# UVA-Computer-Vision-Lab/midvision-probe

Measured on AMD Instinct MI355X. Metric: images/sec feature-extract+probe-step, ViT-B/16 224^2, higher is better.
Workload: dtype f16x2 (compensated fp16 pairs of activations and frozen weights, two f16 MFMA products per contraction, fp32 accumulate, feature error as bf16x3; attention: Q.K^T the same two products over compensated pairs, P.V fp16 probabilities x (fp16 + bf16) V; probe, fp32 residual/LN/softmax/loss as in bf16x3

## Files before the change

midvision-probe_amd/csrc/attention.hip:

```cpp
#include "mvp_common.h"

#ifndef MVP_ATT_NT
#define MVP_ATT_NT 0
#endif
#ifndef MVP_ATT_LD_AUX
#define MVP_ATT_LD_AUX 0
#endif
namespace {

#ifndef MVP_ATT_PRIO
#define MVP_ATT_PRIO 0
#endif
#ifndef MVP_ATT_STAGGER
#define MVP_ATT_STAGGER 0
#endif
#if MVP_ATT_PRIO
#define ATT_PRIO(v) __builtin_amdgcn_s_setprio(v)
#else
#define ATT_PRIO(v)
#endif
#ifndef MVP_ATT_ABLATE
#define MVP_ATT_ABLATE 0
#endif
constexpr int TILE = 64 * 128;
constexpr float ATT_DEFER = 6.0f;

template <int SPLIT>
struct AttnState {
  bf16x8_t q_hi[2][2], q_lo[2][2];
  f32x4_t o_acc[4][2];
  float m_run[2], l_run[2];
};

struct AttnBias {
  const float* row[2];
  float scale;
  const float* rel;
  unsigned qoff[2];
  int Kh, Kw, q16, r16;
};

template <int SPLIT, bool LAST, int VF16 = 0, int BIAS = 0>
__device__ __forceinline__ void attn_tile(AttnState<SPLIT>& st, const char* kb, const char* vb, int key0, int N, float cs, int lane,
                                          const AttnBias& ab = AttnBias{}) {
  static_assert(!VF16 || SPLIT == 3, "the fp16-probability form belongs to the bf16x3 mode");
  const int g = lane >> 4, c16 = lane & 15;
  const int nsub = LAST ? min(4, (N - key0 + 15) >> 4) : 4;
  f32x4_t s[4][2];
#pragma unroll
  for (int t = 0; t < 4; ++t)
#pragma unroll
    for (int qt = 0; qt < 2; ++qt) s[t][qt] = f32x4_t{0.f, 0.f, 0.f, 0.f};
  f32x4_t bv[4][2];
  if constexpr (BIAS == 1) {
#pragma unroll
    for (int t = 0; t < 4; ++t)
#pragma unroll
      for (int qt = 0; qt < 2; ++qt)
        bv[t][qt] = (LAST && t >= nsub) ? f32x4_t{0.f, 0.f, 0.f, 0.f} : *(const f32x4_t*)(ab.row[qt] + key0 + t * 16);
  }
  ATT_PRIO(1);
#pragma unroll
  for (int ks = 0; ks < (MVP_ATT_ABLATE == 3 ? 0 : 2); ++ks) {
    const int coff = (((ks << 2) + g) ^ (lane & 7)) << 4;
#pragma unroll
    for (int t = 0; t < 4; ++t) {
      if (LAST && t >= nsub) continue;
      const char* ka = kb + (t * 16 + c16) * 128 + coff;
      const bf16x8_t k_hi = *(const bf16x8_t*)ka;
      if (VF16 == 2) {
        const f16x8_t k_lo = *(const f16x8_t*)(ka + TILE);
        const f16x8_t k_h = __builtin_bit_cast(f16x8_t, k_hi);
#pragma unroll
        for (int qt = 0; qt < 2; ++qt) {
          s[t][qt] = __builtin_amdgcn_mfma_f32_16x16x32_f16(k_lo, __builtin_bit_cast(f16x8_t, st.q_lo[qt][ks]), s[t][qt], 0, 0, 0);
          s[t][qt] = __builtin_amdgcn_mfma_f32_16x16x32_f16(k_h, __builtin_bit_cast(f16x8_t, st.q_hi[qt][ks]), s[t][qt], 0, 0, 0);
        }
        continue;
      }
      if (SPLIT == 3) {
        const bf16x8_t k_lo = *(const bf16x8_t*)(ka + TILE);
#pragma unroll
        for (int qt = 0; qt < 2; ++qt) {
          s[t][qt] = __builtin_amdgcn_mfma_f32_16x16x32_bf16(k_lo, st.q_hi[qt][ks], s[t][qt], 0, 0, 0);
          s[t][qt] = __builtin_amdgcn_mfma_f32_16x16x32_bf16(k_hi, st.q_lo[qt][ks], s[t][qt], 0, 0, 0);
        }
      }
#pragma unroll
      for (int qt = 0; qt < 2; ++qt)
        s[t][qt] = __builtin_amdgcn_mfma_f32_16x16x32_bf16(k_hi, st.q_hi[qt][ks], s[t][qt], 0, 0, 0);
    }
  }
  ATT_PRIO(0);
  if constexpr (BIAS == 1) {
#pragma unroll
    for (int t = 0; t < 4; ++t)
#pragma unroll
      for (int qt = 0; qt < 2; ++qt)
#pragma unroll
        for (int j = 0; j < 4; ++j) s[t][qt][j] = __builtin_fmaf(s[t][qt][j], ab.scale, bv[t][qt][j]);
  }
  if constexpr (BIAS == 2) {
    unsigned k0 = (unsigned)(key0 + g * 4);
    asm volatile("" : "+v"(k0));
    const unsigned Kw4 = (unsigned)ab.Kw << 2, Kh4 = (unsigned)ab.Kh << 2;
    const unsigned q0y = k0 / (unsigned)ab.Kw;
    unsigned ty = q0y << 2, tx = (k0 - q0y * (unsigned)ab.Kw) << 2;
    const char* base = (const char*)ab.rel;
#pragma unroll
    for (int t = 0; t < 4; ++t) {
      if (!(LAST && t >= nsub)) {
        unsigned ky = ty, kx = tx;
#pragma unroll
        for (int j = 0; j < 4; ++j) {
          const bool dead = LAST && (int)k0 + t * 16 + j >= N;
          const unsigned yy = dead ? 0u : ky, xx = (dead ? 0u : kx) + Kh4;
#pragma unroll
          for (int qt = 0; qt < 2; ++qt)
            s[t][qt][j] = __builtin_fmaf(s[t][qt][j], ab.scale, *(const float*)(base + (ab.qoff[qt] + yy)) + *(const float*)(base + (ab.qoff[qt] + xx)));
          kx += 4;
          if (kx == Kw4) {
            kx = 0;
            ky += 4;
          }
        }
      }
      ty += ab.q16;
      tx += ab.r16;
      if (tx >= Kw4) {
        tx -= Kw4;
        ty += 4;
      }
      __builtin_amdgcn_sched_barrier(0);
    }
  }
  const int kbase = key0 + g * 4;
  bf16x8_t p_hi[2][2], p_lo[2][2];
  f16x8_t p_h[2][2];
#pragma unroll
  for (int qt = 0; qt < 2; ++qt) {
    if (VF16 && MVP_ATT_ABLATE != 1) {
      float tmax = -1e30f;
#pragma unroll
      for (int t = 0; t < 4; ++t)
#pragma unroll
        for (int j = 0; j < 4; ++j) {
          if (LAST) s[t][qt][j] = ((kbase + t * 16 + j) < N) ? s[t][qt][j] : -1e30f;
          tmax = fmaxf(tmax, s[t][qt][j]);
        }
      tmax = fmaxf(tmax, __shfl_xor(tmax, 16, 64));
      tmax = fmaxf(tmax, __shfl_xor(tmax, 32, 64));
      if (__builtin_amdgcn_ballot_w64((tmax - st.m_run[qt]) * cs > ATT_DEFER) != 0) {
        const float m_new = fmaxf(st.m_run[qt], tmax);
        const float alpha = __builtin_amdgcn_exp2f((st.m_run[qt] - m_new) * cs);
        st.m_run[qt] = m_new;
        st.l_run[qt] *= alpha;
#pragma unroll
        for (int dt = 0; dt < 4; ++dt) st.o_acc[dt][qt] *= alpha;
      }
      const float mc = st.m_run[qt] * cs;
      float psum = 0.f;
#pragma unroll
      for (int t = 0; t < 4; ++t)
#pragma unroll
        for (int j = 0; j < 4; ++j) {
          const float pv = (LAST && t >= nsub) ? 0.f : __builtin_amdgcn_exp2f(s[t][qt][j] * cs - mc);
          psum += pv;
          p_h[qt][t >> 1][(t & 1) * 4 + j] = (_Float16)pv;
          p_lo[qt][t >> 1][(t & 1) * 4 + j] = (__bf16)pv;
        }
      st.l_run[qt] += psum;
      continue;
    }
    if (MVP_ATT_ABLATE == 1) {
#pragma unroll
      for (int t = 0; t < 4; ++t)
#pragma unroll
        for (int j = 0; j < 4; ++j) {
          p_hi[qt][t >> 1][(t & 1) * 4 + j] = (__bf16)s[t][qt][j];
          if (SPLIT == 3) p_lo[qt][t >> 1][(t & 1) * 4 + j] = (__bf16)(s[t][qt][j] * cs);
        }
      st.l_run[qt] = 1.f;
      continue;
    }
    float tmax = -1e30f;
#pragma unroll
    for (int t = 0; t < 4; ++t)
#pragma unroll
      for (int j = 0; j < 4; ++j) {
        if (LAST) s[t][qt][j] = ((kbase + t * 16 + j) < N) ? s[t][qt][j] : -1e30f;
        tmax = fmaxf(tmax, s[t][qt][j]);
      }
    tmax = fmaxf(tmax, __shfl_xor(tmax, 16, 64));
    tmax = fmaxf(tmax, __shfl_xor(tmax, 32, 64));
    const float m_new = fmaxf(st.m_run[qt], tmax);
    const float alpha = __builtin_amdgcn_exp2f((st.m_run[qt] - m_new) * cs);
    const float mc = m_new * cs;
    st.m_run[qt] = m_new;
    float psum = 0.f;
#pragma unroll
    for (int t = 0; t < 4; ++t)
#pragma unroll
      for (int j = 0; j < 4; ++j) {
        const float pv = (LAST && t >= nsub) ? 0.f : __builtin_amdgcn_exp2f(s[t][qt][j] * cs - mc);
        psum += pv;
        const __bf16 ph = (__bf16)pv;
        p_hi[qt][t >> 1][(t & 1) * 4 + j] = ph;
        if (SPLIT == 3) p_lo[qt][t >> 1][(t & 1) * 4 + j] = (__bf16)(pv - (float)ph);
      }
    st.l_run[qt] = st.l_run[qt] * alpha + psum;
#pragma unroll
    for (int dt = 0; dt < 4; ++dt) st.o_acc[dt][qt] *= alpha;
  }
  const int tr_q = c16 >> 2, tr_p = lane & 3;
  ATT_PRIO(1);
#pragma unroll
  for (int ks = 0; ks < (MVP_ATT_ABLATE == 2 ? 0 : 2); ++ks) {
    if (LAST && 2 * ks >= nsub) continue;
    const int row = ks * 32 + g * 4 + tr_q;
    const int fsw = ((row >> 1) & 3) << 1;
#pragma unroll
    for (int dt = 0; dt < 4; ++dt) {
      const int off = row * 128 + ((((dt << 1) + (tr_p >> 1)) ^ fsw) << 4) + ((tr_p & 1) << 3);
      const bf16x4_t a0 = __builtin_amdgcn_ds_read_tr16_b64_v4bf16((__attribute__((address_space(3))) bf16x4_t*)(vb + off));
      const bf16x4_t a1 = __builtin_amdgcn_ds_read_tr16_b64_v4bf16((__attribute__((address_space(3))) bf16x4_t*)(vb + off + 16 * 128));
      const bf16x8_t v_hi = __builtin_shufflevector(a0, a1, 0, 1, 2, 3, 4, 5, 6, 7);
      if (VF16) {
        const bf16x4_t b0 = __builtin_amdgcn_ds_read_tr16_b64_v4bf16((__attribute__((address_space(3))) bf16x4_t*)(vb + TILE + off));
        const bf16x4_t b1 = __builtin_amdgcn_ds_read_tr16_b64_v4bf16((__attribute__((address_space(3))) bf16x4_t*)(vb + TILE + off + 16 * 128));
        const bf16x8_t v_lo = __builtin_shufflevector(b0, b1, 0, 1, 2, 3, 4, 5, 6, 7);
        const f16x8_t v_h = __builtin_bit_cast(f16x8_t, v_hi);
#pragma unroll
        for (int qt = 0; qt < 2; ++qt) {
          st.o_acc[dt][qt] = __builtin_amdgcn_mfma_f32_16x16x32_bf16(v_lo, p_lo[qt][ks], st.o_acc[dt][qt], 0, 0, 0);
          st.o_acc[dt][qt] = __builtin_amdgcn_mfma_f32_16x16x32_f16(v_h, p_h[qt][ks], st.o_acc[dt][qt], 0, 0, 0);
        }
        continue;
      }
      if (SPLIT == 3) {
        const bf16x4_t b0 = __builtin_amdgcn_ds_read_tr16_b64_v4bf16((__attribute__((address_space(3))) bf16x4_t*)(vb + TILE + off));
        const bf16x4_t b1 = __builtin_amdgcn_ds_read_tr16_b64_v4bf16((__attribute__((address_space(3))) bf16x4_t*)(vb + TILE + off + 16 * 128));
        const bf16x8_t v_lo = __builtin_shufflevector(b0, b1, 0, 1, 2, 3, 4, 5, 6, 7);
#pragma unroll
        for (int qt = 0; qt < 2; ++qt) {
          st.o_acc[dt][qt] = __builtin_amdgcn_mfma_f32_16x16x32_bf16(v_lo, p_hi[qt][ks], st.o_acc[dt][qt], 0, 0, 0);
          st.o_acc[dt][qt] = __builtin_amdgcn_mfma_f32_16x16x32_bf16(v_hi, p_lo[qt][ks], st.o_acc[dt][qt], 0, 0, 0);
        }
      }
#pragma unroll
      for (int qt = 0; qt < 2; ++qt)
        st.o_acc[dt][qt] = __builtin_amdgcn_mfma_f32_16x16x32_bf16(v_hi, p_hi[qt][ks], st.o_acc[dt][qt], 0, 0, 0);
    }
  }
  ATT_PRIO(0);
}

template <int SPLIT>
__device__ __forceinline__ void attn_load_q(AttnState<SPLIT>& st, const mvp_attention_args& p, size_t rowbase, int q0, int h, int lane) {
  const int g = lane >> 4, c16 = lane & 15;
#pragma unroll
  for (int qt = 0; qt < 2; ++qt) {
    const int qrow = min(q0 + qt * 16 + c16, p.N - 1);
    const size_t off = (rowbase + qrow) * p.ld_qkv + h * 64 + g * 8;
#pragma unroll
    for (int ks = 0; ks < 2; ++ks) {
      st.q_hi[qt][ks] = *(const bf16x8_t*)(p.qkv_hi + off + ks * 32);
      if (SPLIT == 3) st.q_lo[qt][ks] = *(const bf16x8_t*)(p.qkv_lo + off + ks * 32);
    }
  }
#pragma unroll
  for (int i = 0; i < 4; ++i)
#pragma unroll
    for (int j = 0; j < 2; ++j) st.o_acc[i][j] = f32x4_t{0.f, 0.f, 0.f, 0.f};
  st.m_run[0] = st.m_run[1] = -1e30f;
  st.l_run[0] = st.l_run[1] = 0.f;
}

template <int SPLIT>
__device__ __forceinline__ void attn_store(AttnState<SPLIT>& st, const mvp_attention_args& p, size_t rowbase, int q0, int h, int lane) {
  const int g = lane >> 4, c16 = lane & 15;
#pragma unroll
  for (int qt = 0; qt < 2; ++qt) {
    float l = st.l_run[qt];
    l += __shfl_xor(l, 16, 64);
    l += __shfl_xor(l, 32, 64);
    const float inv = 1.0f / l;
    const int qrow = q0 + qt * 16 + c16;
    if (qrow >= p.N) continue;
    const bool ilv = p.out_layout == MVP_PAIR_A_ILV32;
    const size_t ob = (rowbase + qrow) * p.ld_out + (ilv ? h * 128 : h * 64) + g * 4;
#pragma unroll
    for (int dt = 0; dt < 4; ++dt) {
      uint32_t h01, l01, h23, l23;
      if (p.out_f16) {
        split2_f16_comp(st.o_acc[dt][qt][0] * inv, st.o_acc[dt][qt][1] * inv, h01, l01);
        split2_f16_comp(st.o_acc[dt][qt][2] * inv, st.o_acc[dt][qt][3] * inv, h23, l23);
      } else {
        split2_bf16(st.o_acc[dt][qt][0] * inv, st.o_acc[dt][qt][1] * inv, h01, l01);
        split2_bf16(st.o_acc[dt][qt][2] * inv, st.o_acc[dt][qt][3] * inv, h23, l23);
      }
      if (ilv) {
        const size_t o = ob + (dt >> 1) * 64 + (dt & 1) * 16;
        store_out((u32x2_t*)(p.out_hi + o), u32x2_t{h01, h23}, MVP_ATT_NT);
        store_out((u32x2_t*)(p.out_hi + o + 32), u32x2_t{l01, l23}, MVP_ATT_NT);
      } else {
        store_out((u32x2_t*)(p.out_hi + ob + dt * 16), u32x2_t{h01, h23}, MVP_ATT_NT);
        if (p.out_lo) store_out((u32x2_t*)(p.out_lo + ob + dt * 16), u32x2_t{l01, l23}, MVP_ATT_NT);
      }
    }
  }
}

template <int SPLIT>
__device__ __forceinline__ void attn_stage_piece(const mvp_attention_args& p, size_t rowbase, int h, int key0, int r, char* kdst, char* vdst, int lane) {
  const int rsub = lane >> 3;
  const int kc = ((lane & 7) ^ rsub) << 3;
  const int vc = ((lane & 7) ^ (((lane >> 4) & 3) << 1)) << 3;
  const int HD = p.H * 64;
  if (MVP_ATT_ABLATE == 4) return;
  const int krow = min(key0 + r + rsub, p.N - 1);
  const size_t ro = (rowbase + krow) * p.ld_qkv + h * 64;
  __builtin_amdgcn_global_load_lds(GLB_PTR(p.qkv_hi + ro + HD + kc), LDS_PTR(kdst + r * 128), 16, 0, MVP_ATT_LD_AUX);
  __builtin_amdgcn_global_load_lds(GLB_PTR(p.qkv_hi + ro + 2 * HD + vc), LDS_PTR(vdst + r * 128), 16, 0, MVP_ATT_LD_AUX);
  if (SPLIT == 3) {
    __builtin_amdgcn_global_load_lds(GLB_PTR(p.qkv_lo + ro + HD + kc), LDS_PTR(kdst + TILE + r * 128), 16, 0, MVP_ATT_LD_AUX);
    __builtin_amdgcn_global_load_lds(GLB_PTR(p.qkv_lo + ro + 2 * HD + vc), LDS_PTR(vdst + TILE + r * 128), 16, 0, MVP_ATT_LD_AUX);
  }
}

template <int BIAS> struct AttnKArgs { typedef mvp_attention_args type; };
template <> struct AttnKArgs<1> { typedef mvp_attention_bias_args type; };
template <> struct AttnKArgs<2> { typedef mvp_attention_relpos_args type; };
__host__ __device__ __forceinline__ const mvp_attention_args& att_of(const mvp_attention_args& a) { return a; }
__host__ __device__ __forceinline__ const mvp_attention_args& att_of(const mvp_attention_bias_args& a) { return a.att; }
__host__ __device__ __forceinline__ const mvp_attention_args& att_of(const mvp_attention_relpos_args& a) { return a.att; }
__device__ __forceinline__ void attn_bias_rows(AttnBias& ab, const mvp_attention_bias_args& a, int bh, int h, int q0, int lane) {
  const int g = lane >> 4, c16 = lane & 15;
#pragma unroll
  for (int qt = 0; qt < 2; ++qt)
    ab.row[qt] = a.bias + (size_t)h * (size_t)a.bias_head_stride + (size_t)min(q0 + qt * 16 + c16, a.att.N - 1) * (size_t)a.ld_bias + g * 4;
}
__device__ __forceinline__ void attn_bias_rows(AttnBias& ab, const mvp_attention_relpos_args& a, int bh, int h, int q0, int lane) {
  const int c16 = lane & 15;
#pragma unroll
  for (int qt = 0; qt < 2; ++qt) ab.qoff[qt] = ((unsigned)min(q0 + qt * 16 + c16, a.att.N - 1) * (unsigned)a.ld_rel) << 2;
}
__device__ __forceinline__ void attn_bias_rows(AttnBias&, const mvp_attention_args&, int, int, int, int) {}
__device__ __forceinline__ void attn_bias_pair(AttnBias& ab, const mvp_attention_relpos_args& a, int bh) { ab.rel = a.rel + (size_t)bh * (size_t)a.rel_bh_stride; }
__device__ __forceinline__ void attn_bias_pair(AttnBias&, const mvp_attention_bias_args&, int) {}
__device__ __forceinline__ void attn_bias_pair(AttnBias&, const mvp_attention_args&, int) {}
__device__ __forceinline__ void attn_bias_init(AttnBias& ab, const mvp_attention_relpos_args& a) {
  ab.Kh = a.Kh;
  ab.Kw = a.Kw;
  ab.q16 = (16 / a.Kw) << 2;
  ab.r16 = (16 % a.Kw) << 2;
}
__device__ __forceinline__ void attn_bias_init(AttnBias&, const mvp_attention_bias_args&) {}
__device__ __forceinline__ void attn_bias_init(AttnBias&, const mvp_attention_args&) {}

template <int SPLIT, int VF16 = 0, int BIAS = 0>
__global__ __launch_bounds__(256) void attention_stream_kernel(const typename AttnKArgs<BIAS>::type pa) {
  const mvp_attention_args& p = att_of(pa);
  f16_saturate_mode();
  extern __shared__ __attribute__((aligned(16))) char smem[];
  constexpr int NARR = (SPLIT == 3) ? 2 : 1;
  constexpr int STAGE = 2 * NARR * TILE;
  const int lane = threadIdx.x & 63, wave = threadIdx.x >> 6;
  const int bh = blockIdx.y, b = bh / p.H, h = bh - b * p.H;
  const int q0 = blockIdx.x * 128 + wave * 32;
  const int nkt = (p.N + 63) >> 6;
  const size_t rowbase = (size_t)b * p.N;
  AttnState<SPLIT> st;
  attn_load_q<SPLIT>(st, p, rowbase, q0, h, lane);
  const float cs = BIAS ? 1.44269504088896340736f : p.scale * 1.44269504088896340736f;
  const bool active = q0 < p.N;
  AttnBias ab{};
  if constexpr (BIAS != 0) {
    ab.scale = p.scale;
    attn_bias_init(ab, pa);
    attn_bias_pair(ab, pa, bh);
    if (active) attn_bias_rows(ab, pa, bh, h, q0, lane);
  }

  auto stage = [&](int buf, int kt) {
    char* base = smem + buf * STAGE;
#pragma unroll
    for (int ps = 0; ps < 2; ++ps) attn_stage_piece<SPLIT>(p, rowbase, h, kt * 64, ps * 32 + wave * 8, base, base + NARR * TILE, lane);
  };
  stage(0, 0);
  asm volatile("s_waitcnt vmcnt(0)" ::: "memory");
  __syncthreads();
  for (int kt = 0; kt < nkt; ++kt) {
    if (kt + 1 < nkt) stage((kt + 1) & 1, kt + 1);
    if (active) {
      const char* kb = smem + (kt & 1) * STAGE;
      if (kt == nkt - 1) attn_tile<SPLIT, true, VF16, BIAS>(st, kb, kb + NARR * TILE, kt * 64, p.N, cs, lane, ab);
      else attn_tile<SPLIT, false, VF16, BIAS>(st, kb, kb + NARR * TILE, kt * 64, p.N, cs, lane, ab);
    }
    asm volatile("s_waitcnt vmcnt(0)" ::: "memory");
    __syncthreads();
  }
  if (active) attn_store<SPLIT>(st, p, rowbase, q0, h, lane);
}

template <int SPLIT, int VF16 = 0, int BIAS = 0>
__global__ __launch_bounds__(512) void attention_resident_kernel(const typename AttnKArgs<BIAS>::type pa) {
  const mvp_attention_args& p = att_of(pa);
  f16_saturate_mode();
  extern __shared__ __attribute__((aligned(16))) char smem[];
  constexpr int NARR = (SPLIT == 3) ? 2 : 1;
  constexpr int STAGE = 2 * NARR * TILE;
  const int lane = threadIdx.x & 63, wave = threadIdx.x >> 6;
  const int q0 = wave * 32;
  const int nkt = (p.N + 63) >> 6, nslot = nkt + 1;
  const int npair = p.B * p.H;
  const float cs = BIAS ? 1.44269504088896340736f : p.scale * 1.44269504088896340736f;
  const bool active = q0 < p.N;
  const int g = lane >> 4, c16 = lane & 15;
  AttnBias ab{};
  if constexpr (BIAS != 0) {
    ab.scale = p.scale;
    attn_bias_init(ab, pa);
  }

  auto stage_tile = [&](int bh, int kt, int slot) {
    const int b = bh / p.H, h = bh - b * p.H;
    char* base = smem + slot * STAGE;
    attn_stage_piece<SPLIT>(p, (size_t)b * p.N, h, kt * 64, wave * 8, base, base + NARR * TILE, lane);
  };
  bf16x8_t qn_hi[2][2], qn_lo[2][2];
  auto fetch_q = [&](int bh) {
    const int b = bh / p.H, h = bh - b * p.H;
#pragma unroll
    for (int qt = 0; qt < 2; ++qt) {
      const int qrow = min(q0 + qt * 16 + c16, p.N - 1);
      const size_t off = ((size_t)b * p.N + qrow) * p.ld_qkv + h * 64 + g * 8;
#pragma unroll
      for (int ks = 0; ks < 2; ++ks) {
        qn_hi[qt][ks] = *(const bf16x8_t*)(p.qkv_hi + off + ks * 32);
        if (SPLIT == 3) qn_lo[qt][ks] = *(const bf16x8_t*)(p.qkv_lo + off + ks * 32);
      }
    }
  };

  int bh = blockIdx.x;
  if (bh >= npair) return;
  stage_tile(bh, 0, 0);
  fetch_q(bh);
  asm volatile("s_waitcnt vmcnt(0)" ::: "memory");
  __syncthreads();
  AttnState<SPLIT> st;
  for (int i = 0; bh < npair; ++i, bh += gridDim.x) {
    const int b = bh / p.H, h = bh - b * p.H;
    const size_t rowbase = (size_t)b * p.N;
    const int s0 = (nkt * i) % nslot;
    if constexpr (BIAS != 0) {
      attn_bias_pair(ab, pa, bh);
      if (active) attn_bias_rows(ab, pa, bh, h, q0, lane);
    }
    for (int kt = 1; kt < nkt; ++kt) stage_tile(bh, kt, (s0 + kt) % nslot);
#pragma unroll
    for (int qt = 0; qt < 2; ++qt)
#pragma unroll
      for (int ks = 0; ks < 2; ++ks) {
        st.q_hi[qt][ks] = qn_hi[qt][ks];
        if (SPLIT == 3) st.q_lo[qt][ks] = qn_lo[qt][ks];
      }
#pragma unroll
    for (int a = 0; a < 4; ++a)
#pragma unroll
      for (int c = 0; c < 2; ++c) st.o_acc[a][c] = f32x4_t{0.f, 0.f, 0.f, 0.f};
    st.m_run[0] = st.m_run[1] = -1e30f;
    st.l_run[0] = st.l_run[1] = 0.f;
    if (active && MVP_ATT_ABLATE != 5) {
      const char* kb = smem + s0 * STAGE;
      if (nkt == 1) attn_tile<SPLIT, true, VF16, BIAS>(st, kb, kb + NARR * TILE, 0, p.N, cs, lane, ab);
      else attn_tile<SPLIT, false, VF16, BIAS>(st, kb, kb + NARR * TILE, 0, p.N, cs, lane, ab);
    }
    asm volatile("s_waitcnt vmcnt(0)" ::: "memory");
    __syncthreads();
    if (MVP_ATT_STAGGER && wave >= 4) __builtin_amdgcn_s_sleep(MVP_ATT_STAGGER);
    const int nbh = bh + gridDim.x;
    if (nbh < npair) {
      stage_tile(nbh, 0, (s0 + nkt) % nslot);
      fetch_q(nbh);
    }
    if (active) {
      for (int kt = 1; kt < (MVP_ATT_ABLATE == 5 ? 0 : nkt); ++kt) {
        const char* kb = smem + ((s0 + kt) % nslot) * STAGE;
        if (kt == nkt - 1) attn_tile<SPLIT, true, VF16, BIAS>(st, kb, kb + NARR * TILE, kt * 64, p.N, cs, lane, ab);
        else attn_tile<SPLIT, false, VF16, BIAS>(st, kb, kb + NARR * TILE, kt * 64, p.N, cs, lane, ab);
      }
    }
    asm volatile("s_waitcnt vmcnt(0)" ::: "memory");
    if (active) attn_store<SPLIT>(st, p, rowbase, q0, h, lane);
    if (nbh < npair) __builtin_amdgcn_s_barrier();
    if (MVP_ATT_STAGGER && wave >= 4) __builtin_amdgcn_s_sleep(MVP_ATT_STAGGER);
  }
}

template <int SPLIT, int VF16 = 0, int BIAS = 0>
int launch_attention(const typename AttnKArgs<BIAS>::type* ka, hipStream_t s) {
  const mvp_attention_args* a = &att_of(*ka);
  constexpr int NARR = (SPLIT == 3) ? 2 : 1;
  constexpr int STAGE = 2 * NARR * TILE;
  constexpr int SMEM_STREAM = 2 * STAGE, SMEM_RES = 5 * STAGE;
  static int configured = [] {
    int e = (int)hipFuncSetAttribute((const void*)attention_stream_kernel<SPLIT, VF16, BIAS>, hipFuncAttributeMaxDynamicSharedMemorySize, SMEM_STREAM);
    if (e == 0) e = (int)hipFuncSetAttribute((const void*)attention_resident_kernel<SPLIT, VF16, BIAS>, hipFuncAttributeMaxDynamicSharedMemorySize, SMEM_RES);
    return e;
  }();
  if (configured != 0) return MVP_ELAUNCH;
  if (a->N <= 256) {
    const int nkt = (a->N + 63) >> 6;
    static const int cus = [] {
      int dev = 0, n = 0;
      if (hipGetDevice(&dev) != hipSuccess || hipDeviceGetAttribute(&n, hipDeviceAttributeMultiprocessorCount, dev) != hipSuccess) n = 0;
      return n > 0 ? n : 256;
    }();
    const int per_cu = (160 * 1024) / ((nkt + 1) * STAGE) > 0 ? (160 * 1024) / ((nkt + 1) * STAGE) : 1;
    const int grid = a->B * a->H < cus * per_cu ? a->B * a->H : cus * per_cu;
    hipLaunchKernelGGL((attention_resident_kernel<SPLIT, VF16, BIAS>), dim3(grid), dim3(512), (nkt + 1) * STAGE, s, *ka);
  } else {
    dim3 grid((a->N + 127) / 128, a->B * a->H);
    hipLaunchKernelGGL((attention_stream_kernel<SPLIT, VF16, BIAS>), grid, dim3(256), SMEM_STREAM, s, *ka);
  }
  MVP_LAUNCH_CHECK();
  return MVP_OK;
}

}

static int attention_check(const mvp_attention_args* a) {
  if (!a || !a->qkv_hi || !a->out_hi) return MVP_EINVAL;
  if (a->B <= 0 || a->N <= 0 || a->H <= 0) return MVP_EINVAL;
  if ((a->ld_qkv & 7) || (a->ld_out & 3) || a->ld_qkv < 3 * a->H * 64 || a->ld_out < a->H * 64) return MVP_EINVAL;
  if (a->out_layout != MVP_PAIR_SEPARATE && (a->out_layout != MVP_PAIR_A_ILV32 || a->precision != MVP_PREC_BF16X3 || a->ld_out < 2 * a->H * 64)) return MVP_EINVAL;
  if (a->precision == MVP_PREC_BF16X3) {
    if (!a->qkv_lo || (!a->out_lo && a->out_layout == MVP_PAIR_SEPARATE)) return MVP_EINVAL;
    if (a->v_format != MVP_ATT_V_F16 && a->v_format != MVP_ATT_V_F16_QK_F16 && a->v_format != MVP_ATT_V_BF16_PAIR) return MVP_EINVAL;
    return MVP_OK;
  }
  if (a->precision != MVP_PREC_BF16 || a->v_format != MVP_ATT_V_BF16_PAIR || a->out_f16) return MVP_EINVAL;
  return MVP_OK;
}

template <int BIAS>
static int attention_dispatch(const typename AttnKArgs<BIAS>::type* ka, hipStream_t s) {
  const mvp_attention_args* a = &att_of(*ka);
  if (a->precision == MVP_PREC_BF16X3) {
    if (a->v_format == MVP_ATT_V_F16) return launch_attention<3, 1, BIAS>(ka, s);
    if (a->v_format == MVP_ATT_V_F16_QK_F16) return launch_attention<3, 2, BIAS>(ka, s);
    return launch_attention<3, 0, BIAS>(ka, s);
  }
  return launch_attention<1, 0, BIAS>(ka, s);
}

extern "C" int mvp_attention_fwd(const mvp_attention_args* a, void* stream) {
  if (attention_check(a) != MVP_OK) return MVP_EINVAL;
  return attention_dispatch<0>(a, (hipStream_t)stream);
}

extern "C" int mvp_attention_bias_fwd(const mvp_attention_bias_args* a, void* stream) {
  if (!a || attention_check(&a->att) != MVP_OK) return MVP_EINVAL;
  if (!a->bias || ((uintptr_t)a->bias & 15)) return MVP_EINVAL;
  const int64_t npad = 64 * (((int64_t)a->att.N + 63) / 64);
  if ((a->ld_bias & 3) || a->ld_bias < npad) return MVP_EINVAL;
  if (a->bias_head_stride < (int64_t)a->att.N * a->ld_bias || (a->bias_head_stride & 3)) return MVP_EINVAL;
  return attention_dispatch<1>(a, (hipStream_t)stream);
}

extern "C" int mvp_attention_relpos_fwd(const mvp_attention_relpos_args* a, void* stream) {
  if (!a || attention_check(&a->att) != MVP_OK) return MVP_EINVAL;
  if (!a->rel || ((uintptr_t)a->rel & 3)) return MVP_EINVAL;
  if (a->Kh <= 0 || a->Kw <= 0 || (int64_t)a->Kh * a->Kw != (int64_t)a->att.N) return MVP_EINVAL;
  if ((int64_t)a->ld_rel < (int64_t)a->Kh + a->Kw || a->rel_bh_stride < (int64_t)a->att.N * a->ld_rel) return MVP_EINVAL;
  if ((int64_t)a->att.N * a->ld_rel >= (1ll << 30)) return MVP_EINVAL;
  return attention_dispatch<2>(a, (hipStream_t)stream);
}
```

Before: 11320.

## Specialize attention tail tile by live count and split tail work across blocks

```diff
diff --git a/midvision-probe_amd/csrc/attention.hip b/midvision-probe_amd/csrc/attention.hip
--- a/midvision-probe_amd/csrc/attention.hip
+++ b/midvision-probe_amd/csrc/attention.hip
@@ -21,6 +21,15 @@
 #endif
 #ifndef MVP_ATT_ABLATE
 #define MVP_ATT_ABLATE 0
+#endif
+#ifndef MVP_ATT_PREFETCH2
+#define MVP_ATT_PREFETCH2 0
+#endif
+#ifndef MVP_ATT_NSUB_CONST
+#define MVP_ATT_NSUB_CONST 1
+#endif
+#ifndef MVP_ATT_TAIL_SPLIT
+#define MVP_ATT_TAIL_SPLIT 1
 #endif
 constexpr int TILE = 64 * 128;
 constexpr float ATT_DEFER = 6.0f;
@@ -40,12 +49,16 @@
   int Kh, Kw, q16, r16;
 };
 
-template <int SPLIT, bool LAST, int VF16 = 0, int BIAS = 0>
+template <int SPLIT, bool LAST, int VF16 = 0, int BIAS = 0, int NSUB = 0>
 __device__ __forceinline__ void attn_tile(AttnState<SPLIT>& st, const char* kb, const char* vb, int key0, int N, float cs, int lane,
                                           const AttnBias& ab = AttnBias{}) {
   static_assert(!VF16 || SPLIT == 3, "the fp16-probability form belongs to the bf16x3 mode");
   const int g = lane >> 4, c16 = lane & 15;
-  const int nsub = LAST ? min(4, (N - key0 + 15) >> 4) : 4;
+  constexpr bool CNS = LAST && NSUB != 0;
+  static_assert(NSUB >= 0 && NSUB < 4 && (NSUB == 0 || (LAST && BIAS == 0)), "a constant live count belongs to the unbiased LAST tile");
+  const int nsub = CNS ? NSUB : LAST ? min(4, (N - key0 + 15) >> 4) : 4;
+  auto dead = [](int t) { return CNS && t >= NSUB; };
+  auto masked = [](int t) { return LAST && (!CNS || t == NSUB - 1); };
   f32x4_t s[4][2];
 #pragma unroll
   for (int t = 0; t < 4; ++t)
@@ -145,7 +158,8 @@
       for (int t = 0; t < 4; ++t)
 #pragma unroll
         for (int j = 0; j < 4; ++j) {
-          if (LAST) s[t][qt][j] = ((kbase + t * 16 + j) < N) ? s[t][qt][j] : -1e30f;
+          if (dead(t)) continue;
+          if (masked(t)) s[t][qt][j] = ((kbase + t * 16 + j) < N) ? s[t][qt][j] : -1e30f;
           tmax = fmaxf(tmax, s[t][qt][j]);
         }
       tmax = fmaxf(tmax, __shfl_xor(tmax, 16, 64));
@@ -164,6 +178,11 @@
       for (int t = 0; t < 4; ++t)
 #pragma unroll
         for (int j = 0; j < 4; ++j) {
+          if (dead(t)) {
+            p_h[qt][t >> 1][(t & 1) * 4 + j] = (_Float16)0.f;
+            p_lo[qt][t >> 1][(t & 1) * 4 + j] = (__bf16)0.f;
+            continue;
+          }
           const float pv = (LAST && t >= nsub) ? 0.f : __builtin_amdgcn_exp2f(s[t][qt][j] * cs - mc);
           psum += pv;
           p_h[qt][t >> 1][(t & 1) * 4 + j] = (_Float16)pv;
@@ -188,7 +207,8 @@
     for (int t = 0; t < 4; ++t)
 #pragma unroll
       for (int j = 0; j < 4; ++j) {
-        if (LAST) s[t][qt][j] = ((kbase + t * 16 + j) < N) ? s[t][qt][j] : -1e30f;
+        if (dead(t)) continue;
+        if (masked(t)) s[t][qt][j] = ((kbase + t * 16 + j) < N) ? s[t][qt][j] : -1e30f;
         tmax = fmaxf(tmax, s[t][qt][j]);
       }
     tmax = fmaxf(tmax, __shfl_xor(tmax, 16, 64));
@@ -202,6 +222,11 @@
     for (int t = 0; t < 4; ++t)
 #pragma unroll
       for (int j = 0; j < 4; ++j) {
+        if (dead(t)) {
+          p_hi[qt][t >> 1][(t & 1) * 4 + j] = (__bf16)0.f;
+          if (SPLIT == 3) p_lo[qt][t >> 1][(t & 1) * 4 + j] = (__bf16)0.f;
+          continue;
+        }
         const float pv = (LAST && t >= nsub) ? 0.f : __builtin_amdgcn_exp2f(s[t][qt][j] * cs - mc);
         psum += pv;
         const __bf16 ph = (__bf16)pv;
@@ -403,7 +428,23 @@
   if (active) attn_store<SPLIT>(st, p, rowbase, q0, h, lane);
 }
 
-template <int SPLIT, int VF16 = 0, int BIAS = 0>
+__device__ __forceinline__ bool att_tail_split(int npair, int G) {
+  const int full = npair / G, R = npair - full * G;
+  return MVP_ATT_TAIL_SPLIT && full >= 1 && R > 0 && 2 * R <= G && 16 * ((R - 1) >> 3) + 8 + ((R - 1) & 7) < G;
+}
+__device__ __forceinline__ int att_item(int i, int wg, int wave, int npair, int G, bool split, int& q0) {
+  const int full = npair / G, R = npair - full * G;
+  q0 = wave * 32;
+  if (i < full) return wg + i * G;
+  if (i > full) return -1;
+  if (!split) return wg < R ? full * G + wg : -1;
+  const int t = ((wg >> 4) << 3) + (wg & 7);
+  if (t >= R) return -1;
+  q0 = wave < 4 ? ((wg >> 3) & 1) * 128 + wave * 32 : 256;
+  return full * G + t;
+}
+
+template <int SPLIT, int VF16 = 0, int BIAS = 0, int NSUB_LAST = 0>
 __global__ __launch_bounds__(512) void attention_resident_kernel(const typename AttnKArgs<BIAS>::type pa) {
   const mvp_attention_args& p = att_of(pa);
   f16_saturate_mode();
@@ -411,12 +452,12 @@
   constexpr int NARR = (SPLIT == 3) ? 2 : 1;
   constexpr int STAGE = 2 * NARR * TILE;
   const int lane = threadIdx.x & 63, wave = threadIdx.x >> 6;
-  const int q0 = wave * 32;
   const int nkt = (p.N + 63) >> 6, nslot = nkt + 1;
+  const int npf = (MVP_ATT_PREFETCH2 && nkt > 1) ? 2 : 1;
   const int npair = p.B * p.H;
   const float cs = BIAS ? 1.44269504088896340736f : p.scale * 1.44269504088896340736f;
-  const bool active = q0 < p.N;
   const int g = lane >> 4, c16 = lane & 15;
+  const bool split = att_tail_split(npair, (int)gridDim.x);
   AttnBias ab{};
   if constexpr (BIAS != 0) {
     ab.scale = p.scale;
@@ -429,7 +470,7 @@
     attn_stage_piece<SPLIT>(p, (size_t)b * p.N, h, kt * 64, wave * 8, base, base + NARR * TILE, lane);
   };
   bf16x8_t qn_hi[2][2], qn_lo[2][2];
-  auto fetch_q = [&](int bh) {
+  auto fetch_q = [&](int bh, int q0) {
     const int b = bh / p.H, h = bh - b * p.H;
 #pragma unroll
     for (int qt = 0; qt < 2; ++qt) {
@@ -443,22 +484,24 @@
     }
   };
 
-  int bh = blockIdx.x;
-  if (bh >= npair) return;
-  stage_tile(bh, 0, 0);
-  fetch_q(bh);
+  if ((int)blockIdx.x >= npair) return;
+  int q0, q0n;
+  int bh = att_item(0, blockIdx.x, wave, npair, gridDim.x, split, q0);
+  for (int kt = 0; kt < npf; ++kt) stage_tile(bh, kt, kt);
+  fetch_q(bh, q0);
   asm volatile("s_waitcnt vmcnt(0)" ::: "memory");
   __syncthreads();
   AttnState<SPLIT> st;
-  for (int i = 0; bh < npair; ++i, bh += gridDim.x) {
+  for (int i = 0; bh >= 0; ++i) {
     const int b = bh / p.H, h = bh - b * p.H;
     const size_t rowbase = (size_t)b * p.N;
+    const bool active = q0 < p.N;
     const int s0 = (nkt * i) % nslot;
     if constexpr (BIAS != 0) {
       attn_bias_pair(ab, pa, bh);
       if (active) attn_bias_rows(ab, pa, bh, h, q0, lane);
     }
-    for (int kt = 1; kt < nkt; ++kt) stage_tile(bh, kt, (s0 + kt) % nslot);
+    for (int kt = npf; kt < nkt; ++kt) stage_tile(bh, kt, (s0 + kt) % nslot);
 #pragma unroll
     for (int qt = 0; qt < 2; ++qt)
 #pragma unroll
@@ -474,29 +517,42 @@
     st.l_run[0] = st.l_run[1] = 0.f;
     if (active && MVP_ATT_ABLATE != 5) {
       const char* kb = smem + s0 * STAGE;
-      if (nkt == 1) attn_tile<SPLIT, true, VF16, BIAS>(st, kb, kb + NARR * TILE, 0, p.N, cs, lane, ab);
+      if (nkt == 1) attn_tile<SPLIT, true, VF16, BIAS, NSUB_LAST>(st, kb, kb + NARR * TILE, 0, p.N, cs, lane, ab);
       else attn_tile<SPLIT, false, VF16, BIAS>(st, kb, kb + NARR * TILE, 0, p.N, cs, lane, ab);
     }
     asm volatile("s_waitcnt vmcnt(0)" ::: "memory");
     __syncthreads();
     if (MVP_ATT_STAGGER && wave >= 4) __builtin_amdgcn_s_sleep(MVP_ATT_STAGGER);
-    const int nbh = bh + gridDim.x;
-    if (nbh < npair) {
+    const int nbh = att_item(i + 1, blockIdx.x, wave, npair, gridDim.x, split, q0n);
+    if (nbh >= 0) {
       stage_tile(nbh, 0, (s0 + nkt) % nslot);
-      fetch_q(nbh);
+      if (npf > 1) stage_tile(nbh, 1, s0);
+      fetch_q(nbh, q0n);
     }
     if (active) {
       for (int kt = 1; kt < (MVP_ATT_ABLATE == 5 ? 0 : nkt); ++kt) {
         const char* kb = smem + ((s0 + kt) % nslot) * STAGE;
-        if (kt == nkt - 1) attn_tile<SPLIT, true, VF16, BIAS>(st, kb, kb + NARR * TILE, kt * 64, p.N, cs, lane, ab);
+        if (kt == nkt - 1) attn_tile<SPLIT, true, VF16, BIAS, NSUB_LAST>(st, kb, kb + NARR * TILE, kt * 64, p.N, cs, lane, ab);
         else attn_tile<SPLIT, false, VF16, BIAS>(st, kb, kb + NARR * TILE, kt * 64, p.N, cs, lane, ab);
       }
     }
     asm volatile("s_waitcnt vmcnt(0)" ::: "memory");
     if (active) attn_store<SPLIT>(st, p, rowbase, q0, h, lane);
-    if (nbh < npair) __builtin_amdgcn_s_barrier();
+    if (nbh >= 0) __builtin_amdgcn_s_barrier();
     if (MVP_ATT_STAGGER && wave >= 4) __builtin_amdgcn_s_sleep(MVP_ATT_STAGGER);
-  }
+    bh = nbh;
+    q0 = q0n;
+  }
+}
+
+template <int SPLIT, int VF16, int BIAS, int NSUB_LAST>
+int launch_resident(const typename AttnKArgs<BIAS>::type* ka, int grid, int smem, hipStream_t s) {
+  constexpr int SMEM_RES = 5 * 2 * ((SPLIT == 3) ? 2 : 1) * TILE;
+  static int configured = (int)hipFuncSetAttribute((const void*)attention_resident_kernel<SPLIT, VF16, BIAS, NSUB_LAST>,
+                                                   hipFuncAttributeMaxDynamicSharedMemorySize, SMEM_RES);
+  if (configured != 0) return MVP_ELAUNCH;
+  hipLaunchKernelGGL((attention_resident_kernel<SPLIT, VF16, BIAS, NSUB_LAST>), dim3(grid), dim3(512), smem, s, *ka);
+  return MVP_OK;
 }
 
 template <int SPLIT, int VF16 = 0, int BIAS = 0>
@@ -504,13 +560,7 @@
   const mvp_attention_args* a = &att_of(*ka);
   constexpr int NARR = (SPLIT == 3) ? 2 : 1;
   constexpr int STAGE = 2 * NARR * TILE;
-  constexpr int SMEM_STREAM = 2 * STAGE, SMEM_RES = 5 * STAGE;
-  static int configured = [] {
-    int e = (int)hipFuncSetAttribute((const void*)attention_stream_kernel<SPLIT, VF16, BIAS>, hipFuncAttributeMaxDynamicSharedMemorySize, SMEM_STREAM);
-    if (e == 0) e = (int)hipFuncSetAttribute((const void*)attention_resident_kernel<SPLIT, VF16, BIAS>, hipFuncAttributeMaxDynamicSharedMemorySize, SMEM_RES);
-    return e;
-  }();
-  if (configured != 0) return MVP_ELAUNCH;
+  constexpr int SMEM_STREAM = 2 * STAGE;
   if (a->N <= 256) {
     const int nkt = (a->N + 63) >> 6;
     static const int cus = [] {
@@ -520,8 +570,21 @@
     }();
     const int per_cu = (160 * 1024) / ((nkt + 1) * STAGE) > 0 ? (160 * 1024) / ((nkt + 1) * STAGE) : 1;
     const int grid = a->B * a->H < cus * per_cu ? a->B * a->H : cus * per_cu;
-    hipLaunchKernelGGL((attention_resident_kernel<SPLIT, VF16, BIAS>), dim3(grid), dim3(512), (nkt + 1) * STAGE, s, *ka);
+    const int smem = (nkt + 1) * STAGE;
+    const int nsub = (BIAS == 0 && MVP_ATT_NSUB_CONST) ? (((a->N - 1) & 63) >> 4) + 1 : 4;
+    int e;
+    if constexpr (BIAS == 0) {
+      e = nsub == 1   ? launch_resident<SPLIT, VF16, BIAS, 1>(ka, grid, smem, s)
+          : nsub == 2 ? launch_resident<SPLIT, VF16, BIAS, 2>(ka, grid, smem, s)
+          : nsub == 3 ? launch_resident<SPLIT, VF16, BIAS, 3>(ka, grid, smem, s)
+                      : launch_resident<SPLIT, VF16, BIAS, 0>(ka, grid, smem, s);
+    } else {
+      e = launch_resident<SPLIT, VF16, BIAS, 0>(ka, grid, smem, s);
+    }
+    if (e != MVP_OK) return e;
   } else {
+    static int configured = (int)hipFuncSetAttribute((const void*)attention_stream_kernel<SPLIT, VF16, BIAS>, hipFuncAttributeMaxDynamicSharedMemorySize, SMEM_STREAM);
+    if (configured != 0) return MVP_ELAUNCH;
     dim3 grid((a->N + 127) / 128, a->B * a->H);
     hipLaunchKernelGGL((attention_stream_kernel<SPLIT, VF16, BIAS>), grid, dim3(256), SMEM_STREAM, s, *ka);
   }
```

Result: no change. 11410 (median of 6 runs) (+0.8%).
